# JackAILab/ConsistentID

Hardware: AMD Instinct MI355X
Metric: 512x512 SD1.5 images/sec/node @50 DDIM steps (higher is better)
Workload: dtype f16; 1 GPU; sd15 ConsistentID 512x512, 50 DDIM steps, batch 4/GPU (global 4), CFG batch 8, LoRA rank 128 merged, start_merge_step 30, hipGraph on; global_batch=4, parallelism=dp1 (images sharded, no in-step collective)

## Files before the change

consistentid_amd/csrc/attn.hip:

```cpp
#include "common.h"
#include "../../include/cid.h"
#include <stdlib.h>
#include <type_traits>

#ifndef CID_ATTN_ABL
#define CID_ATTN_ABL 0
#endif
#ifdef CID_ATTN_MAX_AT_HEAD
#define CID_ATTN_HEADMAX true
#else
#define CID_ATTN_HEADMAX false
#endif

namespace {

__device__ __forceinline__ float max17f(float m, const f32x16& v) {
#pragma unroll
    for (int r = 0; r < 16; r += 2) m = __builtin_fmaxf(__builtin_fmaxf(m, v[r]), v[r + 1]);
    return m;
}

template <int D, int QT, int NWV>
struct AttnCfg {
    static constexpr int NT = 64 * NWV;
    static constexpr int BQ = 32 * QT * NWV;
    static constexpr int DKP = (D + 15) / 16 * 16;
    static constexpr int KSTEPS = DKP / 16;
    static constexpr int DVT = (D + 31) / 32;
    static constexpr int NCH = D / 8;
    static constexpr int CR = DVT * 32 - D;
    static constexpr int KBYTES = (DKP / 8) * 1024;
    static constexpr int VDATA = D * 128;
    static constexpr int VBYTES = VDATA + CR * 128;
    static constexpr int BUF = KBYTES + VBYTES;
    static constexpr int PPW = (NCH + NWV - 1) / NWV;
};

template <int D, int QT, int NWV, bool MASK, bool CAUSAL = false>
__global__ void __launch_bounds__(64 * NWV, (QT == 1 && D <= 40 && NWV == 4) ? 3 : ((QT == 1 && D <= 80) ? 2 : 1))
self_attn_kernel(const half_t* __restrict__ q, const half_t* __restrict__ k, const half_t* __restrict__ vt,
                 half_t* __restrict__ out, int N, int heads, int ldq, int ldk, int dvp, int ldo, int n_keys, int xcd_remap) {
#if defined(__HIP_DEVICE_COMPILE__)
    using Cfg = AttnCfg<D, QT, NWV>;
    constexpr int NT = Cfg::NT, KSTEPS = Cfg::KSTEPS, DVT = Cfg::DVT;
    constexpr int NCH = Cfg::NCH, CR = Cfg::CR;
    extern __shared__ __attribute__((aligned(16))) char smem[];
    typedef __attribute__((address_space(3))) void lds_void;

    const int tid = threadIdx.x, lane = tid & 63;
    const int wave = __builtin_amdgcn_readfirstlane(tid >> 6);
    const int idx = lane & 31, hi = lane >> 5;
    int bid = blockIdx.x + gridDim.x * (blockIdx.y + gridDim.y * blockIdx.z);
    {
        const int nwg = gridDim.x * gridDim.y * gridDim.z;
        if (xcd_remap && (nwg & 7) == 0) bid = (bid & 7) * (nwg >> 3) + (bid >> 3);
    }
    const int bx = bid % (int)gridDim.x;
    const int h = (bid / (int)gridDim.x) % (int)gridDim.y, b = bid / (int)(gridDim.x * gridDim.y);
    const int q0 = bx * Cfg::BQ + wave * (32 * QT);

    const half_t* kbase = k + (long)b * N * ldk + h * D;
    const half_t* vbase = vt + ((long)(b * heads + h) * dvp) * N;

#if defined(CID_ATTN_NOBIAS)
    constexpr bool BIAS = false;
#else
    constexpr bool BIAS = Cfg::DKP > D;
#endif
    static_assert(!BIAS || Cfg::DKP - D == 8, "pad is one 16-byte slot");
    static_assert(!(CAUSAL && BIAS), "causal mode: the running max starts behind the mask (no bias slot)");
    if (Cfg::DKP > D) {
        half8 pad = zero_h8();
        if (BIAS) pad[0] = (half_t)1.f;
        for (int r = tid; r < 2 * 64; r += NT)
            *reinterpret_cast<half8*>(smem + (r >> 6) * Cfg::BUF + NCH * 1024 + (r & 63) * 16) = pad;
    }
    const bool bias_lane = BIAS && ((KSTEPS - 1) * 16 + hi * 8 == D);

    half8 qf[QT][KSTEPS];
#pragma unroll
    for (int t = 0; t < QT; ++t) {
        const half_t* qrow = q + ((long)b * N + q0 + t * 32 + idx) * ldq + h * D;
#pragma unroll
        for (int kk = 0; kk < KSTEPS; ++kk) {
            const int c = kk * 16 + hi * 8;
            qf[t][kk] = (c < D) ? ld_global_h8(qrow + c) : zero_h8();
        }
    }

    constexpr bool ONES = (D % 32) != 0;
    constexpr int ONES_REG = ((D % 32) & 3) + 4 * ((D % 32) >> 3);
    constexpr int ONES_HI = ((D % 32) >> 2) & 1;
    if (ONES) {
        half8 one;
#pragma unroll
        for (int i = 0; i < 8; ++i) one[i] = (half_t)1.f;
        for (int e = tid; e < 2 * 8 * CR; e += NT) {
            const int bf = e / (8 * CR), rem = e - bf * (8 * CR);
            *reinterpret_cast<half8*>(smem + bf * Cfg::BUF + Cfg::KBYTES + Cfg::VDATA + rem * 16) = one;
        }
    }

    const __amdgpu_buffer_rsrc_t rs_k = __builtin_amdgcn_make_buffer_rsrc((void*)kbase, 0, (unsigned)(((long)(N - 1) * ldk + D) * 2), 0x00020000);
    const __amdgpu_buffer_rsrc_t rs_v = __builtin_amdgcn_make_buffer_rsrc((void*)vbase, 0, (unsigned)((long)D * N * 2), 0x00020000);
    const unsigned kvo = (unsigned)(lane * ldk * 2);
    unsigned vvo[Cfg::PPW];
#pragma unroll
    for (int j = 0; j < Cfg::PPW; ++j) {
        const int sl = (j * NWV + wave) * 64 + lane;
        const int c = sl / D, r = sl - c * D;
        vvo[j] = (unsigned)(((long)r * N + c * 8) * 2);
    }
    auto dma_k = [&](int key0, int buf) {
#pragma unroll
        for (int j = 0; j < Cfg::PPW; ++j) {
            const int p = j * NWV + wave;
            if (p < NCH)
                __builtin_amdgcn_raw_ptr_buffer_load_lds(rs_k, (lds_void*)(smem + buf * Cfg::BUF + p * 1024), 16, kvo,
                                                         key0 * ldk * 2 + p * 16, 0, 0);
        }
    };
    auto dma_v = [&](int key0, int buf) {
#pragma unroll
        for (int j = 0; j < Cfg::PPW; ++j) {
            const int p = j * NWV + wave;
            if (p < NCH)
                __builtin_amdgcn_raw_ptr_buffer_load_lds(rs_v, (lds_void*)(smem + buf * Cfg::BUF + Cfg::KBYTES + p * 1024), 16,
                                                         vvo[j], key0 * 2, 0, 0);
        }
    };
    auto qk = [&](int buf, f32x16 (&s)[2][QT]) {
        const char* kb = smem + buf * Cfg::BUF;
#pragma unroll
        for (int kt = 0; kt < 2; ++kt)
#pragma unroll
            for (int t = 0; t < QT; ++t) s[kt][t] = zero_f16v();
#pragma unroll
        for (int kk = 0; kk < KSTEPS; ++kk) {
            half8 kf[2];
#pragma unroll
            for (int kt = 0; kt < 2; ++kt)
                kf[kt] = *reinterpret_cast<const half8*>(kb + (kk * 2 + hi) * 1024 + (kt * 32 + idx) * 16);
#pragma unroll
            for (int kt = 0; kt < 2; ++kt)
#pragma unroll
                for (int t = 0; t < QT; ++t) { if (!(CID_ATTN_ABL & 4)) s[kt][t] = mfma32(kf[kt], qf[t][kk], s[kt][t]); else s[kt][t][kk] += (float)kf[kt][0]; }
        }
    };
    const int vlane = (hi * D + idx) * 16;
    const int vlane_c = Cfg::VDATA + (hi * CR + idx + (DVT - 1) * 32 - D) * 16;
    const bool vconst_lane = (DVT - 1) * 32 + idx >= D;

    f32x16 oacc[DVT][QT];
#pragma unroll
    for (int d = 0; d < DVT; ++d)
#pragma unroll
        for (int t = 0; t < QT; ++t) oacc[d][t] = zero_f16v();
    float m_run[QT], l_run[QT];
#pragma unroll
    for (int t = 0; t < QT; ++t) { m_run[t] = -INFINITY; l_run[t] = 0.f; }

    const int ntiles = CAUSAL ? (min(n_keys, bx * Cfg::BQ + Cfg::BQ) + 63) / 64 : N / 64;
    dma_k(0, 0); dma_v(0, 0);
    if (ntiles > 1) dma_k(64, 1);
    asm volatile("s_waitcnt vmcnt(0)" ::: "memory");
    __syncthreads();
    f32x16 s_cur[2][QT], s_nxt[2][QT];
    qk(0, s_cur);
    auto tile_max = [&](f32x16 (&sc)[2][QT], int t) {
        float mx = max17f(sc[0][t][0], sc[0][t]);
        mx = max17f(mx, sc[1][t]);
        return fmaxf(mx, __shfl_xor(mx, 32, 64));
    };
    auto rebias = [&](f32x16 (&sc)[2][QT], int t, float m_new, float delta) {
        if (bias_lane) qf[t][KSTEPS - 1][0] = (half_t)(-m_new);
#pragma unroll
        for (int kt = 0; kt < 2; ++kt)
#pragma unroll
            for (int r = 0; r < 16; ++r) sc[kt][t][r] -= delta;
    };
    float mx_a[QT], mx_b[QT];
    if (MASK && BIAS && n_keys < 64) {
#pragma unroll
        for (int kt = 0; kt < 2; ++kt)
#pragma unroll
            for (int t = 0; t < QT; ++t)
#pragma unroll
                for (int r = 0; r < 16; ++r)
                    if (kt * 32 + crow(r, hi) >= n_keys) s_cur[kt][t][r] = -INFINITY;
    }
#pragma unroll
    for (int t = 0; t < QT; ++t) {
        const float mx = tile_max(s_cur, t);
        if (BIAS) {
            const float m0 = (float)(half_t)fminf(fmaxf(mx, -60000.f), 60000.f);
            rebias(s_cur, t, m0, m0);
            m_run[t] = m0;
            mx_a[t] = mx - m0;
        } else {
            mx_a[t] = mx;
        }
        mx_b[t] = 0.f;
    }
    __syncthreads();

    auto step = [&](int tile, auto has_next_tag, f32x16 (&s_cur)[2][QT], f32x16 (&s_nxt)[2][QT], float (&mx_cur)[QT],
                    float (&mx_nxt)[QT]) {
        constexpr bool HAS_NEXT = decltype(has_next_tag)::value;
        const int cur = tile & 1;
        if (!(CID_ATTN_ABL & 8)) {
            if (tile + 2 < ntiles) dma_k((tile + 2) * 64, cur);
            if (HAS_NEXT) dma_v((tile + 1) * 64, cur ^ 1);
        }
        if (MASK && (tile + 1) * 64 > n_keys) {
#pragma unroll
            for (int kt = 0; kt < 2; ++kt)
#pragma unroll
                for (int t = 0; t < QT; ++t)
#pragma unroll
                    for (int r = 0; r < 16; ++r)
                        if (tile * 64 + kt * 32 + crow(r, hi) >= n_keys) s_cur[kt][t][r] = -INFINITY;
        }
        if (CAUSAL && (tile * 64 + 63 > q0 || (tile + 1) * 64 > n_keys)) {
#pragma unroll
            for (int kt = 0; kt < 2; ++kt)
#pragma unroll
                for (int t = 0; t < QT; ++t)
#pragma unroll
                    for (int r = 0; r < 16; ++r) {
                        const int j = tile * 64 + kt * 32 + crow(r, hi);
                        if (j > q0 + t * 32 + idx || j >= n_keys) s_cur[kt][t][r] = -INFINITY;
                    }
        }
#pragma unroll
        for (int t = 0; t < QT; ++t) {
            const float mx = (CID_ATTN_ABL & 16) ? s_cur[0][t][0] : ((MASK || CAUSAL || CID_ATTN_HEADMAX) ? tile_max(s_cur, t) : mx_cur[t]);
            if (__any(mx > (BIAS ? 8.f : m_run[t] + 8.f))) {
                float m_new, alpha;
                if (BIAS) {
                    m_new = (float)(half_t)fminf(m_run[t] + fmaxf(mx, 0.f), 60000.f);
                    const float delta = m_new - m_run[t];
                    alpha = __builtin_amdgcn_exp2f(-delta);
                    rebias(s_cur, t, m_new, delta);
                } else {
                    m_new = fmaxf(m_run[t], mx);
                    alpha = __builtin_amdgcn_exp2f(m_run[t] - m_new);
                }
                m_run[t] = m_new;
                l_run[t] *= alpha;
#pragma unroll
                for (int d = 0; d < DVT; ++d)
#pragma unroll
                    for (int r = 0; r < 16; ++r) oacc[d][t][r] *= alpha;
            }
        }
        if (HAS_NEXT) qk(cur ^ 1, s_nxt);
        half8 pf[QT][4];
#pragma unroll
        for (int t = 0; t < QT; ++t) {
            const float m = m_run[t];
            float rs = 0.f;
#pragma unroll
            for (int kt = 0; kt < 2; ++kt)
#pragma unroll
                for (int g = 0; g < 2; ++g) {
                    half8 pv;
#pragma unroll
                    for (int i = 0; i < 8; ++i) {
                        const float a_ = BIAS ? s_cur[kt][t][g * 8 + i] : s_cur[kt][t][g * 8 + i] - m;
                        const float p = (CID_ATTN_ABL & 1) ? a_ * 0.001f : __builtin_amdgcn_exp2f(a_);
                        if (!ONES) rs += p;
                        pv[i] = (half_t)p;
                    }
                    pf[t][kt * 2 + g] = pv;
                }
            if (!ONES) l_run[t] += rs;
        }
        const char* vb = smem + cur * Cfg::BUF + Cfg::KBYTES;
#pragma unroll
        for (int ks = 0; ks < 4; ++ks) {
            half8 vf[DVT];
#pragma unroll
            for (int d = 0; d < DVT; ++d) {
                int off = vlane + (ks * 2 * D + d * 32) * 16;
                if (CR > 0 && d == DVT - 1) off = vconst_lane ? vlane_c + ks * 2 * CR * 16 : off;
                vf[d] = *reinterpret_cast<const half8*>(vb + off);
            }
#pragma unroll
            for (int d = 0; d < DVT; ++d)
#pragma unroll
                for (int t = 0; t < QT; ++t) { if (!(CID_ATTN_ABL & 2)) oacc[d][t] = mfma32(vf[d], pf[t][ks], oacc[d][t]); else oacc[d][t][ks] += (float)vf[d][0] * (float)pf[t][ks][0]; }
        }
        if (HAS_NEXT && !MASK && !CAUSAL && !CID_ATTN_HEADMAX) {
#pragma unroll
            for (int t = 0; t < QT; ++t) mx_nxt[t] = tile_max(s_nxt, t);
        }
        asm volatile("s_waitcnt vmcnt(0)" ::: "memory");
        __syncthreads();
    };
    int tile = 0;
    for (; tile + 2 < ntiles; tile += 2) {
        step(tile, std::true_type{}, s_cur, s_nxt, mx_a, mx_b);
        step(tile + 1, std::true_type{}, s_nxt, s_cur, mx_b, mx_a);
    }
    if (ntiles - tile == 2) {
        step(tile, std::true_type{}, s_cur, s_nxt, mx_a, mx_b);
        step(tile + 1, std::false_type{}, s_nxt, s_cur, mx_b, mx_a);
    } else {
        step(tile, std::false_type{}, s_cur, s_nxt, mx_a, mx_b);
    }

#pragma unroll
    for (int t = 0; t < QT; ++t) {
        float l;
        if (ONES) {
            const float mine = oacc[DVT - 1][t][ONES_REG];
            const float other = __shfl_xor(mine, 32, 64);
            l = (hi == ONES_HI) ? mine : other;
        } else {
            l = l_run[t] + __shfl_xor(l_run[t], 32, 64);
        }
        const float inv = 1.f / l;
        half_t* orow = out + ((long)b * N + q0 + t * 32 + idx) * ldo + h * D;
#pragma unroll
        for (int d = 0; d < DVT; ++d)
#pragma unroll
            for (int j = 0; j < 4; ++j) {
                const int dd = d * 32 + 8 * j + 4 * hi;
                if (dd < D) {
                    half4 o;
#pragma unroll
                    for (int i = 0; i < 4; ++i) o[i] = (half_t)(oacc[d][t][j * 4 + i] * inv);
                    *reinterpret_cast<half4*>(orow + dd) = o;
                }
            }
    }
#endif
}

template <int D, int QT, int NWV, bool MASK = false, bool CAUSAL = false>
int launch_attn(const half_t* q, const half_t* k, const half_t* vt, half_t* out, int B, int N, int heads,
                int ldq, int ldk, int dvp, int ldo, int n_keys, hipStream_t s) {
    using Cfg = AttnCfg<D, QT, NWV>;
    constexpr int smem = 2 * Cfg::BUF;
    static bool configured = false;
    auto kern = self_attn_kernel<D, QT, NWV, MASK, CAUSAL>;
    if (!configured) {
        hipError_t herr = hipFuncSetAttribute((const void*)kern, hipFuncAttributeMaxDynamicSharedMemorySize, smem);
        if (herr != hipSuccess) {
            cid_set_error("cid_self_attn_f16: cannot reserve %d bytes of LDS (%s)", smem, hipGetErrorString(herr));
            return -5;
        }
        configured = true;
    }
    dim3 grid(N / Cfg::BQ, heads, B);
    static int remap = -1;
    if (remap < 0) { const char* e = getenv("CID_ATTN_XCD"); remap = e ? atoi(e) : 1; }
    hipLaunchKernelGGL(kern, grid, dim3(Cfg::NT), smem, s, q, k, vt, out, N, heads, ldq, ldk, dvp, ldo, n_keys, remap);
    return 0;
}

}

extern "C" int cid_self_attn_f16(const cid_half* q, const cid_half* k, const cid_half* vt, cid_half* out,
                                 int32_t B, int32_t N, int32_t heads, int32_t d,
                                 int32_t ldq, int32_t ldk, int32_t dvp, int32_t ldo, cid_stream_t stream) {
    return cid_self_attn_keys_f16(q, k, vt, out, B, N, heads, d, ldq, ldk, dvp, ldo, N, stream);
}

extern "C" int cid_self_attn_keys_f16(const cid_half* q, const cid_half* k, const cid_half* vt, cid_half* out,
                                      int32_t B, int32_t N, int32_t heads, int32_t d, int32_t ldq, int32_t ldk,
                                      int32_t dvp, int32_t ldo, int32_t n_keys, cid_stream_t stream) {
    CID_CHECK_ARG(q && k && vt && out, "cid_self_attn_f16: null pointer");
    CID_CHECK_ARG(n_keys > 0 && n_keys <= N, "cid_self_attn_keys_f16: n_keys must be in (0, N] (got %d, N = %d)", n_keys, N);
    CID_CHECK_ARG(B > 0 && heads > 0 && N > 0 && N % 64 == 0, "cid_self_attn_f16: N must be a positive multiple of 64 (got %d)", N);
    CID_CHECK_ARG(ldq % 8 == 0 && ldk % 8 == 0 && ldo % 4 == 0 && dvp >= d, "cid_self_attn_f16: bad pitches");
    const half_t* Q = (const half_t*)q; const half_t* K = (const half_t*)k; const half_t* V = (const half_t*)vt;
    half_t* O = (half_t*)out;
    hipStream_t s = (hipStream_t)stream;
    int rc = -22;
#define CID_ATTN(DD, QT, NWV) rc = launch_attn<DD, QT, NWV>(Q, K, V, O, B, N, heads, ldq, ldk, dvp, ldo, n_keys, s)
#define CID_ATTN_MASKED(DD) \
    rc = (N % 128 == 0) ? launch_attn<DD, 1, 4, true>(Q, K, V, O, B, N, heads, ldq, ldk, dvp, ldo, n_keys, s) \
                        : launch_attn<DD, 1, 2, true>(Q, K, V, O, B, N, heads, ldq, ldk, dvp, ldo, n_keys, s)
    if (n_keys != N) {
        if (d == 80) CID_ATTN_MASKED(80);
        else if (d == 64) CID_ATTN_MASKED(64);
        else if (d == 40) CID_ATTN_MASKED(40);
        else if (d == 160) CID_ATTN_MASKED(160);
        else if (d == 32) CID_ATTN_MASKED(32);
        else { cid_set_error("cid_self_attn_keys_f16: unsupported head dim %d (40, 64, 80, 160, 32)", d); return -22; }
        if (rc) return rc;
        CID_CHECK_LAUNCH("cid_self_attn_keys_f16");
        return 0;
    }
    if (d == 40) {
        if (N % 128 == 0) CID_ATTN(40, 1, 4); else CID_ATTN(40, 1, 2);
    } else if (d == 64 || d == 80) {
        static int force_qt = -1;
        if (force_qt < 0) { const char* e = getenv("CID_ATTN_QT"); force_qt = e ? atoi(e) : 0; }
        const bool qt2 = (N % 256 == 0) && force_qt == 2;
        if (d == 64) {
            if (qt2) CID_ATTN(64, 2, 4); else if (N % 128 == 0) CID_ATTN(64, 1, 4); else CID_ATTN(64, 1, 2);
        } else {
            if (qt2) CID_ATTN(80, 2, 4); else if (N % 128 == 0) CID_ATTN(80, 1, 4); else CID_ATTN(80, 1, 2);
        }
    } else if (d == 160) {
        if (N % 128 == 0) CID_ATTN(160, 1, 4); else CID_ATTN(160, 1, 2);
    } else if (d == 32) {
        if (N % 128 == 0) CID_ATTN(32, 1, 4); else CID_ATTN(32, 1, 2);
    } else {
        cid_set_error("cid_self_attn_f16: unsupported head dim %d (40, 64, 80, 160, 32)", d);
        return -22;
    }
#undef CID_ATTN
#undef CID_ATTN_MASKED
    if (rc) return rc;
    CID_CHECK_LAUNCH("cid_self_attn_f16");
    return 0;
}

extern "C" int cid_self_attn_causal_f16(const cid_half* q, const cid_half* k, const cid_half* vt, cid_half* out,
                                        int32_t B, int32_t N, int32_t heads, int32_t d, int32_t ldq, int32_t ldk,
                                        int32_t dvp, int32_t ldo, int32_t n_keys, cid_stream_t stream) {
    CID_CHECK_ARG(q && k && vt && out, "cid_self_attn_causal_f16: null pointer");
    CID_CHECK_ARG(d == 64, "cid_self_attn_causal_f16: unsupported head dim %d (64)", d);
    CID_CHECK_ARG(B > 0 && heads > 0 && N > 0 && N % 64 == 0, "cid_self_attn_causal_f16: N must be a positive multiple of 64 (got %d)", N);
    CID_CHECK_ARG(n_keys > 0 && n_keys <= N, "cid_self_attn_causal_f16: n_keys must be in (0, N] (got %d, N = %d)", n_keys, N);
    CID_CHECK_ARG(ldq % 8 == 0 && ldk % 8 == 0 && ldo % 4 == 0 && dvp >= d && ldq >= heads * d && ldk >= heads * d &&
                  ldo >= heads * d, "cid_self_attn_causal_f16: bad pitches");
    const int rc = launch_attn<64, 1, 2, false, true>((const half_t*)q, (const half_t*)k, (const half_t*)vt, (half_t*)out, B,
                                                      N, heads, ldq, ldk, dvp, ldo, n_keys, (hipStream_t)stream);
    if (rc) return rc;
    CID_CHECK_LAUNCH("cid_self_attn_causal_f16");
    return 0;
}
```

Measured before the change: 7.886 images/s.

## Compute PV tail columns with 16x16 MFMA instead of padded 32-wide tile

For head dims whose remainder modulo 32 is at most 15 (e.g. D=40 in SD1.5), the last output tile of P·V is computed with 16x16x32 MFMAs on a 16-row tail instead of a full 32x32 MFMA padded with constant rows. P fragments are rearranged with permlane16_swap to match the 16x16 layout, and the row-sum is carried in an extra ones column in the tail. This cuts wasted MFMA work and LDS reads on padding, at the cost of extra lane swaps, rescaling shuffles and a more complex epilogue.

```diff
diff --git a/consistentid_amd/csrc/attn.hip b/consistentid_amd/csrc/attn.hip
--- a/consistentid_amd/csrc/attn.hip
+++ b/consistentid_amd/csrc/attn.hip
@@ -20,15 +20,26 @@
     return m;
 }
 
+typedef unsigned u32x4 __attribute__((ext_vector_type(4)));
+__device__ __forceinline__ f32x4 mfma16(half8 a, half8 b, f32x4 c) {
+    return __builtin_amdgcn_mfma_f32_16x16x32_f16(a, b, c, 0, 0, 0);
+}
+
 template <int D, int QT, int NWV>
 struct AttnCfg {
     static constexpr int NT = 64 * NWV;
     static constexpr int BQ = 32 * QT * NWV;
     static constexpr int DKP = (D + 15) / 16 * 16;
     static constexpr int KSTEPS = DKP / 16;
-    static constexpr int DVT = (D + 31) / 32;
+#ifdef CID_ATTN_PV64
+    static constexpr bool TAIL = false;
+#else
+    static constexpr bool TAIL = (D % 32) > 0 && (D % 32) <= 15;
+#endif
+    static constexpr int DVT = TAIL ? D / 32 : (D + 31) / 32;
+    static constexpr int OROWS = DVT * 32 + (TAIL ? 16 : 0);
     static constexpr int NCH = D / 8;
-    static constexpr int CR = DVT * 32 - D;
+    static constexpr int CR = OROWS - D;
     static constexpr int KBYTES = (DKP / 8) * 1024;
     static constexpr int VDATA = D * 128;
     static constexpr int VBYTES = VDATA + CR * 128;
@@ -44,6 +55,7 @@
     using Cfg = AttnCfg<D, QT, NWV>;
     constexpr int NT = Cfg::NT, KSTEPS = Cfg::KSTEPS, DVT = Cfg::DVT;
     constexpr int NCH = Cfg::NCH, CR = Cfg::CR;
+    constexpr bool TAIL = Cfg::TAIL;
     extern __shared__ __attribute__((aligned(16))) char smem[];
     typedef __attribute__((address_space(3))) void lds_void;
 
@@ -97,7 +109,8 @@
         for (int i = 0; i < 8; ++i) one[i] = (half_t)1.f;
         for (int e = tid; e < 2 * 8 * CR; e += NT) {
             const int bf = e / (8 * CR), rem = e - bf * (8 * CR);
-            *reinterpret_cast<half8*>(smem + bf * Cfg::BUF + Cfg::KBYTES + Cfg::VDATA + rem * 16) = one;
+            *reinterpret_cast<half8*>(smem + bf * Cfg::BUF + Cfg::KBYTES + Cfg::VDATA + rem * 16) =
+                (!TAIL || rem % CR == 0) ? one : zero_h8();
         }
     }
 
@@ -150,7 +163,19 @@
     const int vlane = (hi * D + idx) * 16;
     const int vlane_c = Cfg::VDATA + (hi * CR + idx + (DVT - 1) * 32 - D) * 16;
     const bool vconst_lane = (DVT - 1) * 32 + idx >= D;
-
+    constexpr int TR = D % 32;
+    const int tchunk = 2 * ((lane >> 4) & 1) + (lane >> 5);
+    const int vtail = (lane & 15) < TR ? (tchunk * D + DVT * 32 + (lane & 15)) * 16
+                                       : Cfg::VDATA + ((tchunk ^ 1) * CR + (lane & 15) - TR) * 16;
+    const int vtail_step = (lane & 15) < TR ? 4 * D * 16 : 4 * CR * 16;
+
+    f32x4 otail[QT][2];
+    if (TAIL) {
+#pragma unroll
+        for (int t = 0; t < QT; ++t)
+#pragma unroll
+            for (int u = 0; u < 2; ++u) otail[t][u] = f32x4{0.f, 0.f, 0.f, 0.f};
+    }
     f32x16 oacc[DVT][QT];
 #pragma unroll
     for (int d = 0; d < DVT; ++d)
@@ -252,6 +277,15 @@
                 for (int d = 0; d < DVT; ++d)
 #pragma unroll
                     for (int r = 0; r < 16; ++r) oacc[d][t][r] *= alpha;
+                if (TAIL) {
+                    const float alpha_x = __shfl_xor(alpha, 16, 64);
+#pragma unroll
+                    for (int u = 0; u < 2; ++u) {
+                        const float au = (((lane >> 4) & 1) == u) ? alpha : alpha_x;
+#pragma unroll
+                        for (int i = 0; i < 4; ++i) otail[t][u][i] *= au;
+                    }
+                }
             }
         }
         if (HAS_NEXT) qk(cur ^ 1, s_nxt);
@@ -283,13 +317,30 @@
 #pragma unroll
             for (int d = 0; d < DVT; ++d) {
                 int off = vlane + (ks * 2 * D + d * 32) * 16;
-                if (CR > 0 && d == DVT - 1) off = vconst_lane ? vlane_c + ks * 2 * CR * 16 : off;
+                if (!TAIL && CR > 0 && d == DVT - 1) off = vconst_lane ? vlane_c + ks * 2 * CR * 16 : off;
                 vf[d] = *reinterpret_cast<const half8*>(vb + off);
             }
 #pragma unroll
             for (int d = 0; d < DVT; ++d)
 #pragma unroll
                 for (int t = 0; t < QT; ++t) { if (!(CID_ATTN_ABL & 2)) oacc[d][t] = mfma32(vf[d], pf[t][ks], oacc[d][t]); else oacc[d][t][ks] += (float)vf[d][0] * (float)pf[t][ks][0]; }
+        }
+        if (TAIL && !(CID_ATTN_ABL & 2)) {
+#pragma unroll
+            for (int p = 0; p < 2; ++p) {
+                const half8 va = *reinterpret_cast<const half8*>(vb + vtail + p * vtail_step);
+#pragma unroll
+                for (int t = 0; t < QT; ++t) {
+                    u32x4 pa = __builtin_bit_cast(u32x4, pf[t][2 * p]), pb = __builtin_bit_cast(u32x4, pf[t][2 * p + 1]);
+#pragma unroll
+                    for (int w = 0; w < 4; ++w) {
+                        const auto sw = __builtin_amdgcn_permlane16_swap(pa[w], pb[w], false, false);
+                        pa[w] = sw[0]; pb[w] = sw[1];
+                    }
+                    otail[t][0] = mfma16(va, __builtin_bit_cast(half8, pa), otail[t][0]);
+                    otail[t][1] = mfma16(va, __builtin_bit_cast(half8, pb), otail[t][1]);
+                }
+            }
         }
         if (HAS_NEXT && !MASK && !CAUSAL && !CID_ATTN_HEADMAX) {
 #pragma unroll
@@ -313,7 +364,12 @@
 #pragma unroll
     for (int t = 0; t < QT; ++t) {
         float l;
-        if (ONES) {
+        float lt[2];
+        if (TAIL) {
+#pragma unroll
+            for (int u = 0; u < 2; ++u) lt[u] = __shfl(otail[t][u][TR & 3], 16 * (TR >> 2) + (lane & 15), 64);
+            l = (idx >> 4) ? lt[1] : lt[0];
+        } else if (ONES) {
             const float mine = oacc[DVT - 1][t][ONES_REG];
             const float other = __shfl_xor(mine, 32, 64);
             l = (hi == ONES_HI) ? mine : other;
@@ -334,6 +390,17 @@
                     *reinterpret_cast<half4*>(orow + dd) = o;
                 }
             }
+        if (TAIL && 4 * (lane >> 4) < TR) {
+#pragma unroll
+            for (int u = 0; u < 2; ++u) {
+                const float invt = 1.f / lt[u];
+                half4 o;
+#pragma unroll
+                for (int i = 0; i < 4; ++i) o[i] = (half_t)(otail[t][u][i] * invt);
+                *reinterpret_cast<half4*>(out + ((long)b * N + q0 + t * 32 + u * 16 + (lane & 15)) * ldo + h * D + DVT * 32 +
+                                          4 * (lane >> 4)) = o;
+            }
+        }
     }
 #endif
 }
```

Result: no change. 7.932 images/s (median of 6 runs) (+0.6%).
